# LuisCossioUOH/Kinet

Measured on AMD Instinct MI355X. Metric: frames/sec (3x800x1333, 300 obj+track queries) at 1/2/4/8 GPUs; MSDeformAttn ms/call, higher is better.
Workload: dtype bf16; 1 GPU; config2 cfgs/train_deformable.yaml: R-50 Deformable-DETR inference forward, d=256, 4 levels, 6/6 layers, 300 queries, box refine; in_flight_batches=3, launch=HIP graph replay per in-flight slot, graph_check=replays bit-identical to eager (every slot), parallelism=replicas x1

## Files before the change

### include/kinet_ffn.h

```cpp
#ifndef KINET_FFN_H_
#define KINET_FFN_H_

#include "kinet_common.h"

#ifdef __cplusplus
extern "C" {
#endif

int kinet_ffn_pack(const void* W1, const void* W2, void* packed, int D, int F, int dtype,
                   kinet_stream_t stream);

int kinet_ffn_fused(const void* X, int ldx, const void* packed, const float* b1, const float* b2,
                    const float* ln_gamma, const float* ln_beta, float ln_eps, void* Y, int ldy,
                    int M, int D, int F, int dtype, kinet_stream_t stream);

int kinet_ffn_pack_attn(const void* Wo, const void* W1, const void* W2, void* packed, int D, int F,
                        int dtype, kinet_stream_t stream);

int kinet_attn_out_ffn_fused(const void* A, int lda, const void* R, int ldr, const void* packed,
                             const float* bo, const float* ln1_gamma, const float* ln1_beta,
                             float ln1_eps, const float* b1, const float* b2, const float* ln2_gamma,
                             const float* ln2_beta, float ln2_eps, void* Y, int ldy, int M, int D,
                             int F, int dtype, kinet_stream_t stream);

int kinet_bottleneck_pack(const float* W3, const float* W1, const float* s3, const float* s1,
                          void* packed, int D, int F, int DB, int dtype, kinet_stream_t stream);

int kinet_bottleneck_pair(const void* X, int ldx, const void* R, const void* packed, const float* b3,
                          const float* b1, void* Y, void* T, int M, int D, int F, int DB, int dtype,
                          kinet_stream_t stream);

int kinet_bottleneck_pack_ds(const float* W3, const float* Wds, const float* W1, const float* s3,
                             const float* sds, const float* s1, void* packed, int D, int F, int DB,
                             int dtype, kinet_stream_t stream);

int kinet_bottleneck_pair_ds(const void* X, int ldx, const void* X0, int ldx0, const void* packed,
                             const float* b3ds, const float* b1, void* Y, void* T, int M, int D, int F,
                             int DB, int dtype, kinet_stream_t stream);

enum kinet_ffn_problem_field {
    KINET_FFNP_KIND = 0,
    KINET_FFNP_M, KINET_FFNP_D, KINET_FFNP_F, KINET_FFNP_DB,
    KINET_FFNP_FIELDS
};
enum kinet_ffn_plan_field {
    KINET_FFNPL_KERNEL = 0,
    KINET_FFNPL_TILES,
    KINET_FFNPL_GRID, KINET_FFNPL_BLOCK, KINET_FFNPL_WAVES,
    KINET_FFNPL_TILE_ROWS,
    KINET_FFNPL_WG_TILES,
    KINET_FFNPL_WG_PER_CU,
    KINET_FFNPL_LDS,
    KINET_FFNPL_FIELDS
};
enum kinet_ffn_pack_kind { KINET_FFN_PACK_FFN = 0, KINET_FFN_PACK_PAIR, KINET_FFN_PACK_DS, KINET_FFN_PACK_ATTN };

int kinet_ffn_set_debug(int flags);
int kinet_ffn_grid_cap(int max_wgs);
int kinet_ffn_launch_plan(const int* problem, int cus, int* plan_out);
int kinet_ffn_last_kernel(void);
const char* kinet_ffn_kernel_name(int kernel);
int kinet_ffn_pack_map(int kind, int D, int F, int DB, int32_t* out);

#ifdef __cplusplus
}
#endif

#endif
```

### kinet_amd/_native.py

```python
import ctypes
import os

import torch

_LIB_PATH = os.environ.get('KINET_AMD_LIB') or os.path.join(os.path.dirname(os.path.abspath(__file__)), '_lib', 'libkinet_amd.so')

P = ctypes.c_void_p
I = ctypes.c_int
I64 = ctypes.c_int64
F = ctypes.c_float

_SIGS = {
    'kinet_msda_forward': [P, P, P, P, P] + [I] * 10 + [P],
    'kinet_msda_backward': [P] * 9 + [I] * 10 + [P],
    'kinet_msda_backward_workspace_bytes': [I] * 5,
    'kinet_msda_backward_tune': [I] * 5,
    'kinet_msda_backward_debug': [I],
    'kinet_msda_backward_last_kernel': [],
    'kinet_msda_fused_last_kernel': [],
    'kinet_msda_encoder_forward': [P, I64, I64, P, P, P, I, P, P] + [I] * 8 + [P, P],
    'kinet_msda_encoder_plan': [P, I, I, I, P],
    'kinet_msda_encoder_set_strips': [I],
    'kinet_msda_encoder_plan_ex': [P, I, I, I, I, P],
    'kinet_msda_launch_plan': [P, I, P],
    'kinet_msda_encoder_forward_split': [P, I64, I64, P, I64, I64, P, P, P, I, P, P] + [I] * 8 + [P, P],
    'kinet_msda_sample_records': [P, P, P, P, I, I, I, I, I, P, I, P, P, I, I, I, P, I, P],
    'kinet_msda_encoder_forward_records': [P, I64, I64, P, P, I, P] + [I] * 8 + [P, P],
    'kinet_msda_fused_forward': [P, I64, I64, I64, P, P, I, P, I, P, P, P, P] + [I] * 10 + [P, P],
    'kinet_gemm_set_flags': [I],
    'kinet_set_solo_launch': [I],
    'kinet_gemm_force_tile': [I, I],
    'kinet_gemm_last_kernel': [],
    'kinet_gemm_rw_last_config': [P],
    'kinet_gemm_rw_grid_cap': [I],
    'kinet_gemm_plan': [I] * 11 + [P, P],
    'kinet_gemm_rw_plan': [P, I, P, P],
    'kinet_gemm_rw_min_a2_rows': [],
    'kinet_gemm_ksplit': [I] * 4,
    'kinet_gemm_headmajor': [P, P, P] + [I] * 7 + [P, P, I, I, P],
    'kinet_gemm_headmajor_ex': [P, P, P, P] + [I] * 7 + [P, P, I, I, I, P],
    'kinet_gemm_headmajor_split': [P, P, P] + [I] * 7 + [P, P, I, I, I, I, P],
    'kinet_gemm': [P, P, P] + [I] * 7 + [P, P, P, I, I, I, P, I, P],
    'kinet_gemm_ex': [P, P, P, P] + [I] * 7 + [P, P, P, I, I, P, P, F, I, P, P],
    'kinet_conv2d': [P, P, P] + [I] * 12 + [P, P, P, I, I, I, P],
    'kinet_conv2d_ex': [P, P, P] + [I] * 14 + [P, P, P, I, I, I, P],
    'kinet_conv2d_splitk': [P, P, P] + [I] * 12 + [P, P, P, I, I, I, P, I, P],
    'kinet_gemm_splitk': [P, P, P] + [I] * 7 + [P, P, P, I, I, P, P, F, I, P, P, I, P],
    'kinet_ffn_pack': [P, P, P, I, I, I, P],
    'kinet_ffn_set_debug': [I],
    'kinet_ffn_grid_cap': [I],
    'kinet_ffn_launch_plan': [P, I, P],
    'kinet_ffn_last_kernel': [],
    'kinet_ffn_kernel_name': [I],
    'kinet_ffn_pack_map': [I, I, I, I, P],
    'kinet_ffn_fused': [P, I, P, P, P, P, P, F, P, I, I, I, I, I, P],
    'kinet_ffn_pack_attn': [P, P, P, P, I, I, I, P],
    'kinet_attn_out_ffn_fused': [P, I, P, I, P, P, P, P, F, P, P, P, P, F, P, I, I, I, I, I, P],
    'kinet_stem_conv_image': [P, P, P, P, P, I, I, I, I, P],
    'kinet_stem_pool_image': [P, P, P, P, P, I, I, I, I, I, P],
    'kinet_bottleneck_pack': [P, P, P, P, P, I, I, I, I, P],
    'kinet_bottleneck_pair': [P, I, P, P, P, P, P, P, I, I, I, I, I, P],
    'kinet_bottleneck_pack_ds': [P, P, P, P, P, P, P, I, I, I, I, P],
    'kinet_bottleneck_pair_ds': [P, I, P, I, P, P, P, P, P, I, I, I, I, I, P],
    'kinet_layernorm': [P] * 5 + [I, I, F, I, I, P],
    'kinet_groupnorm': [P] * 4 + [I] * 5 + [F, I, P, P],
    'kinet_groupnorm_workspace': [I] * 5,
    'kinet_maxpool2d_3x3s2': [P, P] + [I] * 5 + [P],
    'kinet_pack_image_nhwc': [P, P] + [I] * 5 + [P],
    'kinet_pack_image_kwfold': [P, P] + [I] * 8 + [P],
    'kinet_mha_set_mfma': [I],
    'kinet_mha_launch_plan': [P, P],
    'kinet_mha_last_kernel': [],
    'kinet_mha_core': [P, I, P, I, P, I, P, I] + [I] * 5 + [F, I, P, P],
    'kinet_add': [P, P, P, I64, I, P],
    'kinet_box_refine': [P, P, I, P, P, P, I, I, I, P],
    'kinet_nms': [P, P, P, I, F, P],
    'kinet_sine_position_embed': [P, P, P, P] + [I] * 8 + [F, I64, I, P],
    'kinet_transpose': [P, P, I, I, I64, I64, I, P],
    'kinet_im2col_nhwc': [P, P] + [I] * 13 + [P],
    'kinet_col2im_nhwc': [P, P] + [I] * 13 + [P],
    'kinet_gemm_tn_workspace': [I, I, I],
    'kinet_gemm_tn': [P, P, P, I, I, I, I64, I64, I64, I, I, P, P],
    'kinet_colsum_workspace': [I, I],
    'kinet_colsum': [P, P, I, I, I64, I, I, P, P],
    'kinet_layernorm_backward_workspace': [I, I],
    'kinet_layernorm_backward': [P, P, P, P, P, P, I, I, F, I, P, P],
    'kinet_groupnorm_backward_workspace': [I, I, I, I],
    'kinet_groupnorm_backward': [P, P, P, P, P, P, I, I, I, I, F, I, P, P],
    'kinet_mha_backward_workspace': [I, I, I, I],
    'kinet_mha_backward': [P, I, P, I, P, I, P, I, P, P, P, I, I, I, I, I, F, P, P, F, P, P],
    'kinet_mha_core_dropout': [P, I, P, I, P, I, P, I] + [I] * 5 + [F, I, P, F, P, P],
    'kinet_mha_train_plan': [P, P],
    'kinet_mha_train_calls': [],
    'kinet_mha_train_forward': [P, I, P, I, P, I, P, I, P] + [I] * 5 + [F, P, F, P, P],
    'kinet_mha_train_backward_workspace': [I, I, I],
    'kinet_mha_train_backward': [P, I, P, I, P, I, P, I, P, I, P, P, P, P] + [I] * 5 + [F, P, P, F, P, P],
    'kinet_dropout_mask': [P, I64, F, P, P],
    'kinet_dropout_add_layernorm': [P] * 5 + [I, I, F, F, P, P],
    'kinet_dropout_add_layernorm_backward_workspace': [I, I],
    'kinet_dropout_add_layernorm_backward': [P] * 8 + [I, I, F, F, P, P, P],
    'kinet_dropout_act': [P, P, I64, I, F, P, P],
    'kinet_dropout_act_backward': [P, P, P, I64, I, F, P, P],
    'kinet_msda_prep': [P, I64] + [P] * 5 + [I64, I, I, I, I, P],
    'kinet_msda_prep_backward': [P] * 4 + [I64] + [P] * 4 + [I64, I, I, I, I, P],
    'kinet_inverse_sigmoid': [P, P, I64, F, P],
    'kinet_inverse_sigmoid_backward': [P, P, P, I64, F, P],
    'kinet_two_stage_proposals': [P, I, P, P, P, I, I, P],
# ... 150 lines not shown
```

### kinet_amd/csrc/ffn.hip

```cpp
#include <hip/hip_runtime.h>

#include "../../include/kinet_ffn.h"
#include "common.h"
#include "ffn_plan.h"
#include "gemm_common.h"

namespace kinet {
namespace {

struct FfnArgs {
    const void* X;
    const void* W;
    const float* b1;
    const float* b2;
    const float* ln_g;
    const float* ln_b;
    void* Y;
    float eps;
    int ldx, ldy, M, F;
    int x_bytes, w_bytes, y_bytes;
    int dbg;
    const void* A;
    const void* R;
    const float* bo;
    const float* g1;
    const float* be1;
    float eps1;
    int lda, ldr, a_bytes, r_bytes;
};

thread_local int ffn_debug = 0;
thread_local int ffn_cap = 0;
thread_local int ffn_last = -1;

template <int FAMILY, int D, int RT, int WAVES, int DB = 0, bool PRE = false, int RV = 0>
constexpr FfnKernel ffn_entry() {
    constexpr int i = ffn_kernel_index(FAMILY, D, RT, WAVES, DB, PRE, RV);
    static_assert(i >= 0, "an instantiation the table does not list");
    return kFfnKernels[i];
}
template <int LDS, int ROWS, int NS>
constexpr bool ffn_entry_is(const FfnKernel k) {
    return ffn_kernel_lds(k) == LDS && LDS * k.wg_per_cu <= kFfnLdsLimit && k.tile_rows == ROWS && k.ns == NS;
}

typedef uint32_t u32x2 __attribute__((ext_vector_type(2)));

template <typename T>
__device__ __forceinline__ uint32_t pack2(float a, float b) {
    if constexpr (std::is_same<T, bf16_t>::value) {
        return (uint32_t)f32_to_bf16(a).x | ((uint32_t)f32_to_bf16(b).x << 16);
    } else {
        return (uint32_t)__builtin_bit_cast(uint16_t, (f16_t)a) | ((uint32_t)__builtin_bit_cast(uint16_t, (f16_t)b) << 16);
    }
}

template <typename T>
__device__ __forceinline__ void unpack4(u32x2 u, float* v) {
    if constexpr (std::is_same<T, bf16_t>::value) {
        v[0] = __uint_as_float(u[0] << 16); v[1] = __uint_as_float(u[0] & 0xffff0000u);
        v[2] = __uint_as_float(u[1] << 16); v[3] = __uint_as_float(u[1] & 0xffff0000u);
    } else {
        v[0] = (float)__builtin_bit_cast(f16_t, (uint16_t)(u[0] & 0xffffu));
        v[1] = (float)__builtin_bit_cast(f16_t, (uint16_t)(u[0] >> 16));
        v[2] = (float)__builtin_bit_cast(f16_t, (uint16_t)(u[1] & 0xffffu));
        v[3] = (float)__builtin_bit_cast(f16_t, (uint16_t)(u[1] >> 16));
    }
}

__device__ __forceinline__ u32x4 chunk_swap(u32x2 a, u32x2 b) {
    const auto s0 = __builtin_amdgcn_permlane16_swap(a[0], b[0], false, false);
    const auto s1 = __builtin_amdgcn_permlane16_swap(a[1], b[1], false, false);
    return u32x4{s0[0], s1[0], s0[1], s1[1]};
}
__device__ __forceinline__ int chunk_piece_off(int g) { return (g & 1) ? 4 * g + 12 : 4 * g; }

template <int N>
__device__ __forceinline__ void ffn_wait_vmcnt() {
    asm volatile("s_waitcnt vmcnt(%0)" ::"n"(N) : "memory");
}

__device__ __forceinline__ void ffn_lds_barrier() {
    asm volatile("s_waitcnt lgkmcnt(0)" ::: "memory");
    __builtin_amdgcn_s_barrier();
    asm volatile("" ::: "memory");
}

__device__ __forceinline__ void dma16s(__amdgpu_buffer_rsrc_t r, char* dst, unsigned voff, int soff) {
    __builtin_amdgcn_raw_ptr_buffer_load_lds(r, (lds_ptr_t)dst, 16, voff, soff, 0, 0);
}

template <typename T, int D, int RT, int WAVES>
__global__ __launch_bounds__(WAVES * 64) void ffn_fused_kernel(const FfnArgs p, const int ntiles) {
    using G = FfnGeo<D>;
    constexpr int KS = G::KS, NT = G::NT, FR = G::FR;
    static_assert(FR % WAVES == 0, "whole DMA rounds per chunk");
    constexpr int FRW = FR / WAVES;
    constexpr int XN = RT * KS;
    constexpr int NST = RT * NT / 2;
    static_assert(XN == NST, "one extra-count class");
    constexpr int ROWS = WAVES * 16 * RT;
    constexpr int NS = 4;
    constexpr unsigned OOB = 0x80000000u;
    constexpr int PAR = (FFN_MAX_F + 3 * D) * 4;
    __shared__ __attribute__((aligned(16))) char lds[PAR + NS * G::CHUNK];
    static_assert(ffn_entry_is<sizeof(lds), ROWS, NS>(ffn_entry<FFN_K_FUSED, D, RT, WAVES>()), "ffn_plan.h");
// ... 191 lines not shown
            float mean = 0.f, rstd = 1.f;
            if (ln) {
                s += __shfl_xor(s, 16);
                s += __shfl_xor(s, 32);
                mean = s * (1.f / (float)D);
                float qv = 0.f;
#pragma unroll
                for (int nt = 0; nt < NT; ++nt)
#pragma unroll
                    for (int i = 0; i < 4; ++i) {
                        const float d = acc[rt][nt][i] - mean;
                        qv += d * d;
                    }
                qv += __shfl_xor(qv, 16);
                qv += __shfl_xor(qv, 32);
                rstd = rsqrtf(qv * (1.f / (float)D) + p.eps);
            }
#pragma unroll
            for (int kp = 0; kp < KS; ++kp) {
                const int n0 = 32 * kp + 8 * g;
                float o[8];
#pragma unroll
                for (int i = 0; i < 4; ++i) {
                    o[i] = acc[rt][2 * kp][i];
                    o[4 + i] = acc[rt][2 * kp + 1][i];
                }
                if (ln) {
#pragma unroll
                    for (int e = 0; e < 8; ++e) o[e] = (o[e] - mean) * rstd * pg[n0 + e] + pbe[n0 + e];
                }
                u32x4 w;
#pragma unroll
                for (int e = 0; e < 4; ++e) w[e] = pack2<T>(o[2 * e], o[2 * e + 1]);
                const unsigned off = r < p.M ? ((unsigned)r * (unsigned)p.ldy + (unsigned)n0) * 2u : OOB;
                __builtin_amdgcn_raw_buffer_store_b128(__builtin_bit_cast(u32x4, w), ry, off, 0, 0);
            }
        }
        if (ti + 1 < cnt) {
#pragma unroll
            for (int rt = 0; rt < RT; ++rt)
#pragma unroll
                for (int ks = 0; ks < KS; ++ks) xr[rt][ks] = xn[rt][ks];
        }
    }
}

template <typename T, int D, bool PRE = false, int RV = 0>
__global__ __launch_bounds__(512) void ffn_fused_rt2_kernel(const FfnArgs p, const int ntiles) {
    constexpr int RT = 2, WAVES = 8;
    using G = FfnGeo<D>;
    constexpr int KS = G::KS, NT = G::NT, FR = G::FR;
    static_assert(FR % WAVES == 0, "whole DMA rounds per chunk");
    constexpr int FRW = FR / WAVES;
    constexpr int ROWS = WAVES * 16 * RT;
    constexpr int NS = 3;
    constexpr unsigned OOB = 0x80000000u;
    constexpr int PCH = PRE ? KS * NT / FR : 0;
    static_assert(!PRE || (KS * NT) % FR == 0, "Wo must fill whole ring chunks");
    static_assert(!PRE || (FR % NT == 0 && KS % (FR / NT) == 0), "whole k-steps per Wo chunk");
    constexpr int PAR = (FFN_MAX_F + (PRE ? 6 : 3) * D) * 4;
    __shared__ __attribute__((aligned(16))) char lds[PAR + NS * G::CHUNK];
    static_assert(ffn_entry_is<sizeof(lds), ROWS, NS>(ffn_entry<FFN_K_RT2, D, RT, WAVES, 0, PRE, RV>()), "ffn_plan.h");
    float* const pb1 = reinterpret_cast<float*>(lds);
    float* const pb2 = pb1 + FFN_MAX_F;
    float* const pg = pb2 + D;
    float* const pbe = pg + D;
    float* const pbo = pbe + D;
    float* const pg1 = pbo + D;
    float* const pbe1 = pg1 + D;
    char* const ring = lds + PAR;

    const int P = gridDim.x, bx = blockIdx.x;
    const int cnt = bx < ntiles ? (ntiles - 1 - bx) / P + 1 : 0;
    if (cnt == 0) return;
    const int lane = threadIdx.x & 63;
    const int wave = __builtin_amdgcn_readfirstlane(threadIdx.x >> 6);
    const int g = lane >> 4, c16 = lane & 15;
    const int nch = p.F / 32;
    const bool ln = p.ln_g != nullptr;
    const __amdgpu_buffer_rsrc_t rx = __builtin_amdgcn_make_buffer_rsrc((void*)(PRE ? p.A : p.X), (short)0,
                                                                        PRE ? p.a_bytes : p.x_bytes, 0x00020000);
    const __amdgpu_buffer_rsrc_t rw = __builtin_amdgcn_make_buffer_rsrc((void*)p.W, (short)0, p.w_bytes, 0x00020000);
    const __amdgpu_buffer_rsrc_t ry = __builtin_amdgcn_make_buffer_rsrc(p.Y, (short)0, p.y_bytes, 0x00020000);
    const int ldx = PRE ? p.lda : p.ldx;

    for (int i = threadIdx.x; i < p.F; i += WAVES * 64) pb1[i] = p.b1[i];
    for (int i = threadIdx.x; i < D; i += WAVES * 64) {
        pb2[i] = p.b2[i];
        pg[i] = ln ? p.ln_g[i] : 1.f;
        pbe[i] = ln ? p.ln_b[i] : 0.f;
        if constexpr (PRE) {
            pbo[i] = p.bo[i];
            pg1[i] = p.g1[i];
            pbe1[i] = p.be1[i];
        }
    }
    auto dma_chunk = [&](int q, int c) {
        char* dst = ring + (q % NS) * G::CHUNK;
        const unsigned src = (unsigned)c * (unsigned)G::CHUNK + (unsigned)lane * 16u;
#pragma unroll
        for (int k = 0; k < FRW; ++k) {
            const int f = k * WAVES + wave;
            if constexpr (PRE) {
                dma16s(rw, dst + f * 1024, (unsigned)lane * 16u, c * G::CHUNK + f * 1024);
            } else {
                dma16(rw, dst + f * 1024, src + (unsigned)f * 1024u);
            }
        }
    };
    const int ncht = nch + PCH;
    const int total = cnt * ncht;
    __syncthreads();
    dma_chunk(0, 0);
    if (total > 1) dma_chunk(1, ncht > 1 ? 1 : 0);

    u32x4 xr[RT][KS];
    f32x4 acc[RT][NT];
    for (int ti = 0; ti < cnt; ++ti) {
        const int tile = bx + ti * P;
#pragma unroll
        for (int rt = 0; rt < RT; ++rt) {
            const int r = tile * ROWS + wave * 16 * RT + 16 * rt + c16;
#pragma unroll
            for (int ks = 0; ks < KS; ++ks) {
                const unsigned off = PRE ? (r < p.M ? ((unsigned)r * (unsigned)ldx + (unsigned)(8 * g)) * 2u : OOB) + 64u * ks
                                         : r < p.M ? ((unsigned)r * (unsigned)ldx + (unsigned)(32 * ks + 8 * g)) * 2u : OOB;
                xr[rt][ks] = __builtin_bit_cast(u32x4, __builtin_amdgcn_raw_buffer_load_b128(rx, off, 0, 0));
            }
        }
#pragma unroll
        for (int rt = 0; rt < RT; ++rt)
#pragma unroll
            for (int nt = 0; nt < NT; ++nt) acc[rt][nt] = f32x4{0.f, 0.f, 0.f, 0.f};
        if constexpr (PRE) {
            const __amdgpu_buffer_rsrc_t rr = __builtin_amdgcn_make_buffer_rsrc((void*)p.R, (short)0, p.r_bytes, 0x00020000);
            auto load_res = [&](int kp) {
#pragma unroll
                for (int rt = 0; rt < RT; ++rt) {
                    const int r = tile * ROWS + wave * 16 * RT + 16 * rt + c16;
                    const unsigned off = (r < p.M ? ((unsigned)r * (unsigned)p.ldr + (unsigned)(8 * g)) * 2u : OOB) + 64u * kp;
                    xr[rt][kp] = __builtin_bit_cast(u32x4, __builtin_amdgcn_raw_buffer_load_b128(rr, off, 0, 0));
                }
            };
            constexpr int KPC = FR / NT;
            constexpr int PDW = RV == 1 ? 3 : 4;
#pragma unroll
            for (int u = 0; u < PCH; ++u) {
                const int q = ti * ncht + u;
                if (RV == 1 && u >= 2) ffn_wait_vmcnt<FRW + RT * KPC>();
                else ffn_wait_vmcnt<FRW>();
                ffn_lds_barrier();
                if (q + 2 < total) {
                    int cn = u + 2;
                    if (cn >= ncht) cn -= ncht;
                    dma_chunk(q + 2, cn);
                }
                if constexpr (RV == 1) {
                    if (u > 0) {
#pragma unroll
                        for (int k = 0; k < KPC; ++k) load_res((u - 1) * KPC + k);
                    }
                }
                const char* wb = ring + (q % NS) * G::CHUNK;
                auto frag = [&](int f) { return *reinterpret_cast<const u32x4*>(wb + lane * 16 + f * 1024); };
                u32x4 fo[FR];
#pragma unroll
                for (int f = 0; f < PDW; ++f) fo[f] = frag(f);
#pragma unroll
                for (int f = 0; f < FR; ++f) {
                    if (f + PDW < FR) fo[f + PDW] = frag(f + PDW);
#pragma unroll
                    for (int rt = 0; rt < RT; ++rt) Mma<T>::run(acc[rt][f % NT], fo[f], xr[rt][u * KPC + f / NT]);
                    __builtin_amdgcn_sched_barrier(0);
                }
            }
#pragma unroll
            for (int kp = (RV == 1 ? KS - KPC : 0); kp < KS; ++kp) load_res(kp);
#pragma unroll
            for (int rt = 0; rt < RT; ++rt) {
                asm volatile("" ::: "memory");
                float s = 0.f;
#pragma unroll
                for (int kp = 0; kp < KS; ++kp) {
                    const f32x4 boa = *reinterpret_cast<const f32x4*>(pbo + 32 * kp + 8 * g);
                    const f32x4 bob = *reinterpret_cast<const f32x4*>(pbo + 32 * kp + 8 * g + 4);
                    f32x4 xa, xb;
                    unpack4<T>(u32x2{xr[rt][kp][0], xr[rt][kp][1]}, reinterpret_cast<float*>(&xa));
                    unpack4<T>(u32x2{xr[rt][kp][2], xr[rt][kp][3]}, reinterpret_cast<float*>(&xb));
                    const f32x4 va = acc[rt][2 * kp] + boa + xa;
                    const f32x4 vb = acc[rt][2 * kp + 1] + bob + xb;
                    acc[rt][2 * kp] = va;
                    acc[rt][2 * kp + 1] = vb;
#pragma unroll
                    for (int i = 0; i < 4; ++i) s += va[i] + vb[i];
                }
                s += __shfl_xor(s, 16);
                s += __shfl_xor(s, 32);
                const float mean = s * (1.f / (float)D);
                float qv = 0.f;
#pragma unroll
                for (int nt = 0; nt < NT; ++nt)
#pragma unroll
                    for (int i = 0; i < 4; ++i) {
                        const float d = acc[rt][nt][i] - mean;
                        qv += d * d;
                    }
                qv += __shfl_xor(qv, 16);
                qv += __shfl_xor(qv, 32);
                const float rstd = rsqrtf(qv * (1.f / (float)D) + p.eps1);
#pragma unroll
                for (int kp = 0; kp < KS; ++kp) {
                    const int n0 = 32 * kp + 8 * g;
                    float o[8];
#pragma unroll
                    for (int i = 0; i < 4; ++i) {
                        o[i] = acc[rt][2 * kp][i];
                        o[4 + i] = acc[rt][2 * kp + 1][i];
                    }
#pragma unroll
                    for (int k = 0; k < 8; ++k) o[k] = (o[k] - mean) * rstd * pg1[n0 + k] + pbe1[n0 + k];
#pragma unroll
                    for (int k = 0; k < 4; ++k) xr[rt][kp][k] = pack2<T>(o[2 * k], o[2 * k + 1]);
                    asm volatile("" : "+v"(xr[rt][kp]));
                }
            }
#pragma unroll
            for (int rt = 0; rt < RT; ++rt)
#pragma unroll
                for (int nt = 0; nt < NT; ++nt) acc[rt][nt] = f32x4{0.f, 0.f, 0.f, 0.f};
        }
        for (int c = 0; c < nch; ++c) {
            const int q = ti * ncht + PCH + c;
            if (q + 1 < total) ffn_wait_vmcnt<FRW>();
            else ffn_wait_vmcnt<0>();
            ffn_lds_barrier();
            if (q + 2 < total) {
                int cn = PCH + c + 2;
                if (cn >= ncht) cn -= ncht;
                if (cn >= ncht) cn -= ncht;
                dma_chunk(q + 2, cn);
            }
            const char* wb = ring + (q % NS) * G::CHUNK;
            f32x4 h0[RT], h1[RT];
            {
                const f32x4 bb0 = *reinterpret_cast<const f32x4*>(pb1 + c * 32 + 4 * g);
                const f32x4 bb1 = *reinterpret_cast<const f32x4*>(pb1 + c * 32 + 16 + 4 * g);
#pragma unroll
                for (int rt = 0; rt < RT; ++rt) {
                    h0[rt] = bb0;
                    h1[rt] = bb1;
                }
            }
            auto frag = [&](int f) { return *reinterpret_cast<const u32x4*>(wb + lane * 16 + f * 1024); };
            constexpr int PDA = 2, PDB = 4;
            static_assert(KS >= PDA && NT >= PDB, "prefetch depths");
            u32x4 fa[KS][2], fw[NT];
#pragma unroll
            for (int i = 0; i < PDA; ++i) {
                fa[i][0] = frag(i);
                fa[i][1] = frag(KS + i);
            }
#pragma unroll
            for (int ks = 0; ks < KS; ++ks) {
                if (ks + PDA < KS) {
                    fa[ks + PDA][0] = frag(ks + PDA);
                    fa[ks + PDA][1] = frag(KS + ks + PDA);
                } else {
                    const int t = ks + PDA - KS;
#pragma unroll
                    for (int j = t * PDB / PDA; j < (t + 1) * PDB / PDA; ++j) fw[j] = frag(2 * KS + j);
                }
#pragma unroll
                for (int rt = 0; rt < RT; ++rt) {
                    Mma<T>::run(h0[rt], fa[ks][0], xr[rt][ks]);
                    Mma<T>::run(h1[rt], fa[ks][1], xr[rt][ks]);
                }
                __builtin_amdgcn_sched_barrier(0);
            }
            auto relu = [](float v) { return __builtin_bit_cast(float, max(__builtin_bit_cast(int, v), 0)); };
            u32x4 hb[RT];
#pragma unroll
            for (int rt = 0; rt < RT; ++rt) {
                hb[rt][0] = pack2<T>(relu(h0[rt][0]), relu(h0[rt][1]));
                hb[rt][1] = pack2<T>(relu(h0[rt][2]), relu(h0[rt][3]));
                hb[rt][2] = pack2<T>(relu(h1[rt][0]), relu(h1[rt][1]));
                hb[rt][3] = pack2<T>(relu(h1[rt][2]), relu(h1[rt][3]));
            }
            __builtin_amdgcn_sched_barrier(0);
#pragma unroll
            for (int nt = 0; nt < NT; ++nt) {
                if (nt + PDB < NT) fw[nt + PDB] = frag(2 * KS + nt + PDB);
#pragma unroll
                for (int rt = 0; rt < RT; ++rt) Mma<T>::run(acc[rt][nt], fw[nt], hb[rt]);
                __builtin_amdgcn_sched_barrier(0);
            }
        }
#pragma unroll
        for (int rt = 0; rt < RT; ++rt) {
            const int r = tile * ROWS + wave * 16 * RT + 16 * rt + c16;
            float s = 0.f;
#pragma unroll
            for (int kp = 0; kp < KS; ++kp) {
                float x8[8];
                unpack4<T>(u32x2{xr[rt][kp][0], xr[rt][kp][1]}, x8);
                unpack4<T>(u32x2{xr[rt][kp][2], xr[rt][kp][3]}, x8 + 4);
                const f32x4 b2a = *reinterpret_cast<const f32x4*>(pb2 + 32 * kp + 8 * g);
                const f32x4 b2b = *reinterpret_cast<const f32x4*>(pb2 + 32 * kp + 8 * g + 4);
#pragma unroll
                for (int i = 0; i < 4; ++i) {
                    const float v0 = acc[rt][2 * kp][i] + b2a[i] + x8[i];
                    const float v1 = acc[rt][2 * kp + 1][i] + b2b[i] + x8[4 + i];
                    acc[rt][2 * kp][i] = v0;
                    acc[rt][2 * kp + 1][i] = v1;
                    s += v0 + v1;
                }
            }
            float mean = 0.f, rstd = 1.f;
            if (ln) {
                s += __shfl_xor(s, 16);
                s += __shfl_xor(s, 32);
                mean = s * (1.f / (float)D);
                float qv = 0.f;
#pragma unroll
                for (int nt = 0; nt < NT; ++nt)
#pragma unroll
                    for (int i = 0; i < 4; ++i) {
                        const float d = acc[rt][nt][i] - mean;
                        qv += d * d;
                    }
                qv += __shfl_xor(qv, 16);
                qv += __shfl_xor(qv, 32);
                rstd = rsqrtf(qv * (1.f / (float)D) + p.eps);
            }
#pragma unroll
            for (int kp = 0; kp < KS; ++kp) {
                const int n0 = 32 * kp + 8 * g;
                float o[8];
#pragma unroll
                for (int i = 0; i < 4; ++i) {
                    o[i] = acc[rt][2 * kp][i];
                    o[4 + i] = acc[rt][2 * kp + 1][i];
                }
                if (ln) {
#pragma unroll
                    for (int e = 0; e < 8; ++e) o[e] = (o[e] - mean) * rstd * pg[n0 + e] + pbe[n0 + e];
                }
                u32x4 w;
#pragma unroll
// ... 536 lines not shown
template <typename Args>
int launch_planned(int kind, int M, int D, int F, int DB, int dtype, const Args& a, kinet_stream_t stream) {
    FfnPlan pl;
    if (!ffn_plan(ffn_problem(kind, M, D, F, DB, cu_count()), pl)) return refused(pl);
    ffn_last = pl.kernel;
    constexpr std::make_integer_sequence<int, kNumFfnKernels> all{};
    if (dtype == KINET_BF16) launch_kernel<bf16_t>(pl, (hipStream_t)stream, a, all);
    else launch_kernel<f16_t>(pl, (hipStream_t)stream, a, all);
    KINET_LAUNCH_CHECK();
    return KINET_OK;
}

bool dt16(int dtype) { return dtype == KINET_BF16 || dtype == KINET_F16; }
template <typename... Q>
bool al16(const Q*... q) { return (((uintptr_t)q | ...) & 15u) == 0; }
long long extent(int M, int ld, int D) { return ((long long)(M - 1) * ld + D) * 2; }
constexpr long long k2GiB = 1LL << 31;

}
}

using namespace kinet;

extern "C" int kinet_ffn_set_debug(int flags) {
    const int old = ffn_debug;
    ffn_debug = flags;
    return old;
}

extern "C" int kinet_ffn_grid_cap(int max_wgs) {
    const int old = ffn_cap;
    ffn_cap = max_wgs > 0 ? max_wgs : 0;
    return old;
}

extern "C" int kinet_ffn_last_kernel(void) { return ffn_last; }

extern "C" const char* kinet_ffn_kernel_name(int kernel) {
    return kernel >= 0 && kernel < kNumFfnKernels ? kFfnKernels[kernel].name : nullptr;
}

extern "C" int kinet_ffn_launch_plan(const int* problem, int cus, int* plan_out) {
    KINET_CHECK_ARG(problem != nullptr && plan_out != nullptr && cus > 0, "ffn launch plan: invalid arguments");
    const int* f = problem;
    KINET_CHECK_ARG(f[KINET_FFNP_KIND] >= FFN_FFN && f[KINET_FFNP_KIND] <= FFN_PAIR_DS && f[KINET_FFNP_M] >= 0,
                    "ffn launch plan: invalid problem");
    FfnPlan pl;
    if (!ffn_plan(ffn_problem(f[KINET_FFNP_KIND], f[KINET_FFNP_M], f[KINET_FFNP_D], f[KINET_FFNP_F], f[KINET_FFNP_DB], cus), pl))
        return refused(pl);
    const FfnKernel& k = kFfnKernels[pl.kernel];
    const int rec[KINET_FFNPL_FIELDS] = {pl.kernel, pl.tiles, pl.grid, k.block(), k.waves, k.tile_rows,
                                         k.wg_tiles, k.wg_per_cu, ffn_kernel_lds(k)};
    for (int i = 0; i < KINET_FFNPL_FIELDS; ++i) plan_out[i] = rec[i];
    return KINET_OK;
}

extern "C" int kinet_ffn_pack_map(int kind, int D, int F, int DB, int32_t* out) {
    KINET_CHECK_ARG(kind >= FFN_PACK_FFN && kind <= FFN_PACK_ATTN && out != nullptr, "ffn_pack_map: invalid arguments");
    KINET_CHECK_ARG(D > 0 && D % 32 == 0 && F > 0 && F % 32 == 0 && DB > 0 && DB % 32 == 0,
                    "ffn_pack_map: need D, F, DB multiples of 32 (D=%d F=%d DB=%d)", D, F, DB);
    KINET_CHECK_ARG(DB == D || kind == FFN_PACK_PAIR, "ffn_pack_map: DB must be D but for the bottleneck pair (D=%d DB=%d)", D, DB);
    const long long total = ffn_pack_total(kind, D, F, DB);
    for (long long idx = 0; idx < total; ++idx) {
        const FfnPackSrc e = ffn_pack_src(kind, D, F, DB, idx);
        out[3 * idx] = e.mat;
        out[3 * idx + 1] = e.row;
        out[3 * idx + 2] = e.col;
    }
    return KINET_OK;
}

extern "C" int kinet_ffn_pack(const void* W1, const void* W2, void* packed, int D, int F, int dtype,
                              kinet_stream_t stream) {
    KINET_CHECK_ARG(D > 0 && D % 32 == 0 && F > 0 && F % 32 == 0, "ffn_pack: need D %% 32 == 0 and F %% 32 == 0 (D=%d F=%d)", D, F);
    KINET_CHECK_ARG(dt16(dtype), "ffn_pack: dtype must be bf16 or f16");
    return launch_pack<false>(PackSrc{{W1, W2}, {}}, packed, FFN_PACK_FFN, D, F, D, dtype, stream);
}

extern "C" int kinet_ffn_fused(const void* X, int ldx, const void* packed, const float* b1, const float* b2,
                               const float* ln_gamma, const float* ln_beta, float ln_eps, void* Y, int ldy, int M,
                               int D, int F, int dtype, kinet_stream_t stream) {
    KINET_CHECK_ARG(D == 256 || D == 288, kFfnWhyD, D);
    KINET_CHECK_ARG(F > 0 && F % 32 == 0 && F <= FFN_MAX_F, "ffn_fused: F must be a multiple of 32 in [32, %d] (got %d)", FFN_MAX_F, F);
    KINET_CHECK_ARG(M >= 0 && ldx >= D && ldy >= D && ldx % 8 == 0 && ldy % 8 == 0, "ffn_fused: bad M / ldx / ldy");
    KINET_CHECK_ARG(dt16(dtype), "ffn_fused: dtype must be bf16 or f16");
    KINET_CHECK_ARG(b1 != nullptr && b2 != nullptr, "ffn_fused: b1 and b2 are required");
    KINET_CHECK_ARG((ln_gamma == nullptr) == (ln_beta == nullptr), "ffn_fused: LayerNorm needs both gamma and beta");
    KINET_CHECK_ARG(al16(X, Y, packed, b1, b2, ln_gamma, ln_beta),
                    "ffn_fused: X, Y, packed weights, biases and LayerNorm params must be 16-byte aligned");
    if (M == 0) return KINET_OK;
    const long long xb = extent(M, ldx, D);
    KINET_CHECK_ARG(xb < k2GiB, "ffn_fused: X larger than 2 GiB (split the call)");
    FfnArgs a{};
    a.X = X; a.W = packed; a.b1 = b1; a.b2 = b2; a.ln_g = ln_gamma; a.ln_b = ln_beta; a.Y = Y; a.eps = ln_eps;
    a.ldx = ldx; a.ldy = ldy; a.M = M; a.F = F;
    a.x_bytes = (int)xb;
    a.w_bytes = (int)(ffn_pack_total(FFN_PACK_FFN, D, F, D) * 2);
    const long long yb = extent(M, ldy, D);
    KINET_CHECK_ARG(yb < k2GiB, "ffn_fused: Y larger than 2 GiB (split the call)");
    a.y_bytes = (int)yb;
    a.dbg = ffn_debug;
    return launch_planned(FFN_FFN, M, D, F, D, dtype, a, stream);
}

extern "C" int kinet_ffn_pack_attn(const void* Wo, const void* W1, const void* W2, void* packed, int D, int F,
                                   int dtype, kinet_stream_t stream) {
// ... 109 lines not shown
```

Baseline: 1546 frames/s.

## Stagger FFN wave roles and split weight ring DMA into halves

Splits each weight ring chunk's DMA into W1 and W2 halves issued at different ring steps, so the wait/vmcnt only covers the half about to be read. In the attention-prefixed variant, waves 4-7 lag their second GEMM by one chunk, software-pipelining phase B of chunk c-1 with phase A of chunk c, so the SIMD partner waves alternate between GEMMs. Also switches bf16/f16 packing to a vector convertvector conversion, lowers one residual prefetch depth, and adds a host-queryable schedule description. The aim is less barrier stall and better MFMA overlap, at the cost of more register pressure and a more intricate ring-slot reuse protocol.

```diff
diff --git a/include/kinet_ffn.h b/include/kinet_ffn.h
--- a/include/kinet_ffn.h
+++ b/include/kinet_ffn.h
@@ -55,12 +55,28 @@
 };
 enum kinet_ffn_pack_kind { KINET_FFN_PACK_FFN = 0, KINET_FFN_PACK_PAIR, KINET_FFN_PACK_DS, KINET_FFN_PACK_ATTN };
 
+enum kinet_ffn_sched_field {
+    KINET_FFNS_TOTAL = 0,
+    KINET_FFNS_BARRIERS,
+    KINET_FFNS_BARRIER,
+    KINET_FFNS_SLOT,
+    KINET_FFNS_VMCNT,
+    KINET_FFNS_N_ISSUE,
+    KINET_FFNS_ISSUE,
+    KINET_FFNS_N_EARLY = KINET_FFNS_ISSUE + 6,
+    KINET_FFNS_EARLY,
+    KINET_FFNS_N_READ = KINET_FFNS_EARLY + 6,
+    KINET_FFNS_READ,
+    KINET_FFNS_FIELDS = KINET_FFNS_READ + 6
+};
+
 int kinet_ffn_set_debug(int flags);
 int kinet_ffn_grid_cap(int max_wgs);
 int kinet_ffn_launch_plan(const int* problem, int cus, int* plan_out);
 int kinet_ffn_last_kernel(void);
 const char* kinet_ffn_kernel_name(int kernel);
 int kinet_ffn_pack_map(int kind, int D, int F, int DB, int32_t* out);
+int kinet_ffn_sched(int role, int cnt, int pch, int nch, int q, int half_ops, int* out);
 
 #ifdef __cplusplus
 }
diff --git a/kinet_amd/_native.py b/kinet_amd/_native.py
--- a/kinet_amd/_native.py
+++ b/kinet_amd/_native.py
@@ -53,6 +53,7 @@
     'kinet_ffn_last_kernel': [],
     'kinet_ffn_kernel_name': [I],
     'kinet_ffn_pack_map': [I, I, I, I, P],
+    'kinet_ffn_sched': [I, I, I, I, I, I, P],
     'kinet_ffn_fused': [P, I, P, P, P, P, P, F, P, I, I, I, I, I, P],
     'kinet_ffn_pack_attn': [P, P, P, P, I, I, I, P],
     'kinet_attn_out_ffn_fused': [P, I, P, I, P, P, P, P, F, P, P, P, P, F, P, I, I, I, I, I, P],
diff --git a/kinet_amd/csrc/ffn.hip b/kinet_amd/csrc/ffn.hip
--- a/kinet_amd/csrc/ffn.hip
+++ b/kinet_amd/csrc/ffn.hip
@@ -3,6 +3,7 @@
 #include "../../include/kinet_ffn.h"
 #include "common.h"
 #include "ffn_plan.h"
+#include "ffn_sched.h"
 #include "gemm_common.h"
 
 namespace kinet {
@@ -46,12 +47,17 @@
 
 typedef uint32_t u32x2 __attribute__((ext_vector_type(2)));
 
+typedef float f32x2 __attribute__((ext_vector_type(2)));
+typedef __bf16 bf16x2 __attribute__((ext_vector_type(2)));
+typedef _Float16 f16x2 __attribute__((ext_vector_type(2)));
+
 template <typename T>
 __device__ __forceinline__ uint32_t pack2(float a, float b) {
+    const f32x2 v{a, b};
     if constexpr (std::is_same<T, bf16_t>::value) {
-        return (uint32_t)f32_to_bf16(a).x | ((uint32_t)f32_to_bf16(b).x << 16);
+        return __builtin_bit_cast(uint32_t, __builtin_convertvector(v, bf16x2));
     } else {
-        return (uint32_t)__builtin_bit_cast(uint16_t, (f16_t)a) | ((uint32_t)__builtin_bit_cast(uint16_t, (f16_t)b) << 16);
+        return __builtin_bit_cast(uint32_t, __builtin_convertvector(v, f16x2));
     }
 }
 
@@ -349,8 +355,11 @@
     constexpr int KS = G::KS, NT = G::NT, FR = G::FR;
     static_assert(FR % WAVES == 0, "whole DMA rounds per chunk");
     constexpr int FRW = FR / WAVES;
+    static_assert(FRW % 2 == 0 && 2 * KS == FR / 2, "a chunk is staged as two halves: W1 | W2");
+    constexpr int HW = FRW / 2;
     constexpr int ROWS = WAVES * 16 * RT;
-    constexpr int NS = 3;
+    constexpr int NS = kFfnSchedSlots;
+    static_assert(WAVES == 2 * kFfnSchedRoleSplit, "SIMD partners w, w + 4 take the two roles");
     constexpr unsigned OOB = 0x80000000u;
     constexpr int PCH = PRE ? KS * NT / FR : 0;
     static_assert(!PRE || (KS * NT) % FR == 0, "Wo must fill whole ring chunks");
@@ -392,12 +401,12 @@
             pbe1[i] = p.be1[i];
         }
     }
-    auto dma_chunk = [&](int q, int c) {
-        char* dst = ring + (q % NS) * G::CHUNK;
+    auto dma_half = [&](int q, int c, int half) {
+        char* dst = ring + ffn_sched_slot(q) * G::CHUNK;
         const unsigned src = (unsigned)c * (unsigned)G::CHUNK + (unsigned)lane * 16u;
 #pragma unroll
-        for (int k = 0; k < FRW; ++k) {
-            const int f = k * WAVES + wave;
+        for (int k = 0; k < HW; ++k) {
+            const int f = (half * HW + k) * WAVES + wave;
             if constexpr (PRE) {
                 dma16s(rw, dst + f * 1024, (unsigned)lane * 16u, c * G::CHUNK + f * 1024);
             } else {
@@ -406,10 +415,33 @@
         }
     };
     const int ncht = nch + PCH;
-    const int total = cnt * ncht;
+    const int total = ffn_sched_total(cnt, PCH, nch);
+    auto ring_step = [&](int q, int u, auto extra) {
+        constexpr int EXTRA = decltype(extra)::value;
+        constexpr int MID = ffn_sched_vmcnt(0, 2, HW), END = ffn_sched_vmcnt(0, 1, HW);
+        if (q + 1 < total) ffn_wait_vmcnt<MID + EXTRA>();
+        else ffn_wait_vmcnt<END>();
+        ffn_lds_barrier();
+#pragma unroll
+        for (int i = 0; i < kFfnSchedIssues; ++i) {
+            const int ahead = kFfnSchedIssue[i].chunk;
+            if (q + ahead < total) {
+                int cn = u + ahead;
+                if (cn >= ncht) cn -= ncht;
+                if (cn >= ncht) cn -= ncht;
+                dma_half(q + ahead, cn, kFfnSchedIssue[i].half);
+            }
+        }
+    };
+    using no_extra = std::integral_constant<int, 0>;
     __syncthreads();
-    dma_chunk(0, 0);
-    if (total > 1) dma_chunk(1, ncht > 1 ? 1 : 0);
+    {
+        dma_half(0, 0, FFN_HALF_LO);
+        dma_half(0, 0, FFN_HALF_HI);
+        if (total > 1) dma_half(1, ncht > 1 ? 1 : 0, FFN_HALF_LO);
+    }
+    constexpr bool STAGGER = PRE;
+    const int role = STAGGER ? ffn_sched_role(wave) : 0;
 
     u32x4 xr[RT][KS];
     f32x4 acc[RT][NT];
@@ -440,25 +472,19 @@
                 }
             };
             constexpr int KPC = FR / NT;
-            constexpr int PDW = RV == 1 ? 3 : 4;
+            constexpr int PDW = RV == 1 ? 2 : 4;
 #pragma unroll
             for (int u = 0; u < PCH; ++u) {
                 const int q = ti * ncht + u;
-                if (RV == 1 && u >= 2) ffn_wait_vmcnt<FRW + RT * KPC>();
-                else ffn_wait_vmcnt<FRW>();
-                ffn_lds_barrier();
-                if (q + 2 < total) {
-                    int cn = u + 2;
-                    if (cn >= ncht) cn -= ncht;
-                    dma_chunk(q + 2, cn);
-                }
+                if (RV == 1 && u >= 2) ring_step(q, u, std::integral_constant<int, RT * KPC>{});
+                else ring_step(q, u, no_extra{});
                 if constexpr (RV == 1) {
                     if (u > 0) {
 #pragma unroll
                         for (int k = 0; k < KPC; ++k) load_res((u - 1) * KPC + k);
                     }
                 }
-                const char* wb = ring + (q % NS) * G::CHUNK;
+                const char* wb = ring + ffn_sched_slot(q) * G::CHUNK;
                 auto frag = [&](int f) { return *reinterpret_cast<const u32x4*>(wb + lane * 16 + f * 1024); };
                 u32x4 fo[FR];
 #pragma unroll
@@ -526,46 +552,33 @@
 #pragma unroll
                 for (int nt = 0; nt < NT; ++nt) acc[rt][nt] = f32x4{0.f, 0.f, 0.f, 0.f};
         }
-        for (int c = 0; c < nch; ++c) {
-            const int q = ti * ncht + PCH + c;
-            if (q + 1 < total) ffn_wait_vmcnt<FRW>();
-            else ffn_wait_vmcnt<0>();
-            ffn_lds_barrier();
-            if (q + 2 < total) {
-                int cn = PCH + c + 2;
-                if (cn >= ncht) cn -= ncht;
-                if (cn >= ncht) cn -= ncht;
-                dma_chunk(q + 2, cn);
-            }
-            const char* wb = ring + (q % NS) * G::CHUNK;
+        constexpr int PDA = 2, PDB = 4;
+        static_assert(KS >= PDA && NT >= PDB && PDB > PDA, "prefetch depths");
+        auto slot_of = [&](int q) { return ring + ffn_sched_slot(q) * G::CHUNK; };
+        auto frag = [&](const char* wb, int f) { return *reinterpret_cast<const u32x4*>(wb + lane * 16 + f * 1024); };
+        auto read_a = [&](const char* wb, u32x4(&fa)[KS][2], int ks) {
+            fa[ks][0] = frag(wb, ks);
+            fa[ks][1] = frag(wb, KS + ks);
+        };
+        auto read_bias = [&](int c, f32x4(&bb)[2]) {
+            bb[0] = *reinterpret_cast<const f32x4*>(pb1 + c * 32 + 4 * g);
+            bb[1] = *reinterpret_cast<const f32x4*>(pb1 + c * 32 + 16 + 4 * g);
+        };
+        auto phase_a = [&](const char* wb, const f32x4(&bb)[2], u32x4(&fa)[KS][2], u32x4(&fw)[NT], u32x4(&hb)[RT], auto tail_b) {
             f32x4 h0[RT], h1[RT];
-            {
-                const f32x4 bb0 = *reinterpret_cast<const f32x4*>(pb1 + c * 32 + 4 * g);
-                const f32x4 bb1 = *reinterpret_cast<const f32x4*>(pb1 + c * 32 + 16 + 4 * g);
-#pragma unroll
-                for (int rt = 0; rt < RT; ++rt) {
-                    h0[rt] = bb0;
-                    h1[rt] = bb1;
-                }
-            }
-            auto frag = [&](int f) { return *reinterpret_cast<const u32x4*>(wb + lane * 16 + f * 1024); };
-            constexpr int PDA = 2, PDB = 4;
-            static_assert(KS >= PDA && NT >= PDB, "prefetch depths");
-            u32x4 fa[KS][2], fw[NT];
-#pragma unroll
-            for (int i = 0; i < PDA; ++i) {
-                fa[i][0] = frag(i);
-                fa[i][1] = frag(KS + i);
+#pragma unroll
+            for (int rt = 0; rt < RT; ++rt) {
+                h0[rt] = bb[0];
+                h1[rt] = bb[1];
             }
 #pragma unroll
             for (int ks = 0; ks < KS; ++ks) {
                 if (ks + PDA < KS) {
-                    fa[ks + PDA][0] = frag(ks + PDA);
-                    fa[ks + PDA][1] = frag(KS + ks + PDA);
-                } else {
+                    read_a(wb, fa, ks + PDA);
+                } else if constexpr (decltype(tail_b)::value) {
                     const int t = ks + PDA - KS;
 #pragma unroll
-                    for (int j = t * PDB / PDA; j < (t + 1) * PDB / PDA; ++j) fw[j] = frag(2 * KS + j);
+                    for (int j = t * PDB / PDA; j < (t + 1) * PDB / PDA; ++j) fw[j] = frag(wb, 2 * KS + j);
                 }
 #pragma unroll
                 for (int rt = 0; rt < RT; ++rt) {
@@ -575,7 +588,6 @@
                 __builtin_amdgcn_sched_barrier(0);
             }
             auto relu = [](float v) { return __builtin_bit_cast(float, max(__builtin_bit_cast(int, v), 0)); };
-            u32x4 hb[RT];
 #pragma unroll
             for (int rt = 0; rt < RT; ++rt) {
                 hb[rt][0] = pack2<T>(relu(h0[rt][0]), relu(h0[rt][1]));
@@ -584,13 +596,60 @@
                 hb[rt][3] = pack2<T>(relu(h1[rt][2]), relu(h1[rt][3]));
             }
             __builtin_amdgcn_sched_barrier(0);
+        };
+        auto phase_b = [&](const char* ws, const char* wn, int cn, f32x4(&bb)[2], u32x4(&fa)[KS][2], u32x4(&fw)[NT],
+                           const u32x4(&hb)[RT], auto next_a) {
 #pragma unroll
             for (int nt = 0; nt < NT; ++nt) {
-                if (nt + PDB < NT) fw[nt + PDB] = frag(2 * KS + nt + PDB);
+                if (nt + PDB < NT) {
+                    fw[nt + PDB] = frag(ws, 2 * KS + nt + PDB);
+                } else if constexpr (decltype(next_a)::value) {
+                    const int t = nt + PDB - NT;
+                    if (t < PDA) read_a(wn, fa, t);
+                    else if (t == PDA) read_bias(cn, bb);
+                }
 #pragma unroll
                 for (int rt = 0; rt < RT; ++rt) Mma<T>::run(acc[rt][nt], fw[nt], hb[rt]);
                 __builtin_amdgcn_sched_barrier(0);
             }
+        };
+        const int q0 = ti * ncht + PCH;
+        if (ffn_sched_b_lag(role) == 0) {
+            for (int c = 0; c < nch; ++c) {
+                ring_step(q0 + c, PCH + c, no_extra{});
+                const char* wb = slot_of(q0 + c);
+                u32x4 fa[KS][2], fw[NT], hb[RT];
+                f32x4 bb[2];
+                read_bias(c, bb);
+#pragma unroll
+                for (int i = 0; i < PDA; ++i) read_a(wb, fa, i);
+                phase_a(wb, bb, fa, fw, hb, std::true_type{});
+                phase_b(wb, wb, 0, bb, fa, fw, hb, std::false_type{});
+            }
+        } else {
+            u32x4 fa[KS][2], fw[NT], hb[RT];
+            f32x4 bb[2];
+            ring_step(q0, PCH, no_extra{});
+            {
+                const char* wb = slot_of(q0);
+                read_bias(0, bb);
+#pragma unroll
+                for (int i = 0; i < PDA; ++i) read_a(wb, fa, i);
+                phase_a(wb, bb, fa, fw, hb, std::false_type{});
+            }
+            for (int c = 1; c < nch; ++c) {
+                const char* wp = slot_of(q0 + c - 1);
+#pragma unroll
+                for (int j = 0; j < PDB; ++j) fw[j] = frag(wp, 2 * KS + j);
+                ring_step(q0 + c, PCH + c, no_extra{});
+                const char* wb = slot_of(q0 + c);
+                phase_b(wp, wb, c, bb, fa, fw, hb, std::true_type{});
+                phase_a(wb, bb, fa, fw, hb, std::false_type{});
+            }
+            const char* wl = slot_of(q0 + nch - 1);
+#pragma unroll
+            for (int j = 0; j < PDB; ++j) fw[j] = frag(wl, 2 * KS + j);
+            phase_b(wl, wl, 0, bb, fa, fw, hb, std::false_type{});
         }
 #pragma unroll
         for (int rt = 0; rt < RT; ++rt) {
@@ -1233,6 +1292,32 @@
     const int rec[KINET_FFNPL_FIELDS] = {pl.kernel, pl.tiles, pl.grid, k.block(), k.waves, k.tile_rows,
                                          k.wg_tiles, k.wg_per_cu, ffn_kernel_lds(k)};
     for (int i = 0; i < KINET_FFNPL_FIELDS; ++i) plan_out[i] = rec[i];
+    return KINET_OK;
+}
+
+extern "C" int kinet_ffn_sched(int role, int cnt, int pch, int nch, int q, int half_ops, int* out) {
+    KINET_CHECK_ARG(out != nullptr && (role == 0 || role == 1) && cnt > 0 && pch >= 0 && nch > 0 && half_ops > 0,
+                    "ffn_sched: invalid arguments");
+    const int total = ffn_sched_total(cnt, pch, nch);
+    KINET_CHECK_ARG(q >= -1 && q < total, "ffn_sched: chunk %d outside [-1, %d)", q, total);
+    for (int i = 0; i < KINET_FFNS_FIELDS; ++i) out[i] = -1;
+    out[KINET_FFNS_TOTAL] = total;
+    out[KINET_FFNS_BARRIERS] = ffn_sched_barriers(role, cnt, pch, nch);
+    auto put = [&](int n_field, int field, const FfnHalfList& l) {
+        out[n_field] = l.n;
+        for (int i = 0; i < l.n; ++i) {
+            out[field + 2 * i] = l.e[i].chunk;
+            out[field + 2 * i + 1] = l.e[i].half;
+        }
+    };
+    put(KINET_FFNS_N_ISSUE, KINET_FFNS_ISSUE, ffn_sched_issue(q, total));
+    out[KINET_FFNS_N_EARLY] = out[KINET_FFNS_N_READ] = 0;
+    if (q < 0) return KINET_OK;
+    out[KINET_FFNS_BARRIER] = q;
+    out[KINET_FFNS_SLOT] = ffn_sched_slot(q);
+    out[KINET_FFNS_VMCNT] = ffn_sched_vmcnt(q, total, half_ops);
+    put(KINET_FFNS_N_EARLY, KINET_FFNS_EARLY, ffn_sched_early_reads(role, q, pch, nch));
+    put(KINET_FFNS_N_READ, KINET_FFNS_READ, ffn_sched_reads(role, q, pch, nch));
     return KINET_OK;
 }
 
diff --git a/kinet_amd/csrc/ffn_sched.h b/kinet_amd/csrc/ffn_sched.h
--- /dev/null
+++ b/kinet_amd/csrc/ffn_sched.h
@@ -0,0 +1,71 @@
+#pragma once
+
+namespace kinet {
+
+constexpr int kFfnSchedSlots = 3;
+constexpr int kFfnSchedRoleSplit = 4;
+
+enum FfnHalf { FFN_HALF_LO = 0, FFN_HALF_HI = 1 };
+
+struct FfnChunkHalf {
+    int chunk, half;
+};
+constexpr int kFfnSchedMaxIssue = 3, kFfnSchedMaxRead = 3;
+struct FfnHalfList {
+    int n;
+    FfnChunkHalf e[3];
+};
+
+constexpr int ffn_sched_total(int cnt, int pch, int nch) { return cnt * (pch + nch); }
+constexpr int ffn_sched_slot(int q) { return q % kFfnSchedSlots; }
+constexpr int ffn_sched_role(int wave) { return wave < kFfnSchedRoleSplit ? 0 : 1; }
+constexpr int ffn_sched_b_lag(int role) { return role; }
+
+constexpr FfnChunkHalf kFfnSchedIssue[2] = {{1, FFN_HALF_HI}, {2, FFN_HALF_LO}};
+constexpr int kFfnSchedIssues = 2;
+
+constexpr FfnHalfList ffn_sched_issue(int q, int total) {
+    FfnHalfList l{};
+    if (q < 0) {
+        for (int b = -2; b < 0; ++b)
+            for (int i = 0; i < kFfnSchedIssues; ++i) {
+                const int c = b + kFfnSchedIssue[i].chunk;
+                if (c >= 0 && c < total) l.e[l.n++] = FfnChunkHalf{c, kFfnSchedIssue[i].half};
+            }
+        return l;
+    }
+    for (int i = 0; i < kFfnSchedIssues; ++i) {
+        const int c = q + kFfnSchedIssue[i].chunk;
+        if (c < total) l.e[l.n++] = FfnChunkHalf{c, kFfnSchedIssue[i].half};
+    }
+    return l;
+}
+
+constexpr int ffn_sched_vmcnt(int q, int total, int half_ops) { return q + 1 < total ? half_ops : 0; }
+
+constexpr int ffn_sched_pre(int q, int pch, int nch) { return q % (pch + nch) < pch ? q % (pch + nch) : -1; }
+constexpr int ffn_sched_hidden(int q, int pch, int nch) { return q % (pch + nch) < pch ? -1 : q % (pch + nch) - pch; }
+
+constexpr FfnHalfList ffn_sched_reads(int role, int q, int pch, int nch) {
+    FfnHalfList l{};
+    const int c = ffn_sched_hidden(q, pch, nch), lag = ffn_sched_b_lag(role);
+    if (c < 0 || lag == 0) {
+        l.e[l.n++] = FfnChunkHalf{q, FFN_HALF_LO};
+        l.e[l.n++] = FfnChunkHalf{q, FFN_HALF_HI};
+        return l;
+    }
+    if (c > 0) l.e[l.n++] = FfnChunkHalf{q - 1, FFN_HALF_HI};
+    l.e[l.n++] = FfnChunkHalf{q, FFN_HALF_LO};
+    if (c == nch - 1) l.e[l.n++] = FfnChunkHalf{q, FFN_HALF_HI};
+    return l;
+}
+
+constexpr FfnHalfList ffn_sched_early_reads(int role, int q, int pch, int nch) {
+    FfnHalfList l{};
+    if (ffn_sched_b_lag(role) > 0 && ffn_sched_hidden(q, pch, nch) > 0) l.e[l.n++] = FfnChunkHalf{q - 1, FFN_HALF_HI};
+    return l;
+}
+
+constexpr int ffn_sched_barriers(int , int cnt, int pch, int nch) { return ffn_sched_total(cnt, pch, nch); }
+
+}
```

After: 1568 frames/s (median of 6 runs). 1.01x the previous value.
